# nimiq/snark-setup

Measured on NVIDIA B200. Metric: phase1 contribute+verify G1+G2 powers/sec at 2^22 (1/2/4/8 B200), bit-exact, higher is better.
Workload: dtype u32

## Files before the change

snark-setup_b200/csrc/fp.cuh:

```cuda
#pragma once
#include "ptx.cuh"

namespace ss {

template <class P>
struct Fp {
    static constexpr int N = P::N;
    using Params = P;
#ifndef SS_CALL_GROUP_OPS_LIMBS
#define SS_CALL_GROUP_OPS_LIMBS 12
#endif
    static constexpr bool CALL_GROUP_OPS = (N > SS_CALL_GROUP_OPS_LIMBS);
    uint32_t l[N];

    SS_HD static Fp zero() {
        Fp r;
#pragma unroll
        for (int i = 0; i < N; i++) r.l[i] = 0;
        return r;
    }
    SS_HD static Fp one() {
        Fp r;
#pragma unroll
        for (int i = 0; i < N; i++) r.l[i] = P::one(i);
        return r;
    }
    SS_HD bool is_zero() const {
        uint32_t t = 0;
#pragma unroll
        for (int i = 0; i < N; i++) t |= l[i];
        return t == 0;
    }
    SS_HD bool operator==(const Fp& o) const {
        uint32_t t = 0;
#pragma unroll
        for (int i = 0; i < N; i++) t |= l[i] ^ o.l[i];
        return t == 0;
    }
    SS_HD bool operator!=(const Fp& o) const { return !(*this == o); }
};

#if defined(__CUDACC__)
static __device__ __constant__ uint32_t kOpaqueOnes = 0xffffffffu;
#else
static const uint32_t kOpaqueOnes = 0xffffffffu;
#endif
SS_HD uint32_t opaque_neg(uint32_t x) { return (x ^ kOpaqueOnes) + 1u; }
#if defined(SS_NO_P0_TRICK)
#define SS_P0_TRICK false
#else
#define SS_P0_TRICK true
#endif

template <class P>
SS_HD void fp_final_sub(uint32_t* a) {
    constexpr int N = P::N;
    uint32_t t[N];
    t[0] = sub_cc(a[0], P::mod(0));
#pragma unroll
    for (int i = 1; i < N; i++) t[i] = subc_cc(a[i], P::mod(i));
    uint32_t borrow = subc(0, 0);
#pragma unroll
    for (int i = 0; i < N; i++) a[i] = borrow ? a[i] : t[i];
}

template <class P>
SS_HD Fp<P> fp_add(const Fp<P>& a, const Fp<P>& b) {
    constexpr int N = P::N;
    Fp<P> r;
    r.l[0] = add_cc(a.l[0], b.l[0]);
#pragma unroll
    for (int i = 1; i < N - 1; i++) r.l[i] = addc_cc(a.l[i], b.l[i]);
    r.l[N - 1] = addc(a.l[N - 1], b.l[N - 1]);
    fp_final_sub<P>(r.l);
    return r;
}

template <class P>
SS_HD Fp<P> fp_add_nr(const Fp<P>& a, const Fp<P>& b) {
    constexpr int N = P::N;
    Fp<P> r;
    r.l[0] = add_cc(a.l[0], b.l[0]);
#pragma unroll
    for (int i = 1; i < N - 1; i++) r.l[i] = addc_cc(a.l[i], b.l[i]);
    r.l[N - 1] = addc(a.l[N - 1], b.l[N - 1]);
    return r;
}

template <class P>
SS_HD Fp<P> fp_sub(const Fp<P>& a, const Fp<P>& b) {
    constexpr int N = P::N;
    Fp<P> r;
    r.l[0] = sub_cc(a.l[0], b.l[0]);
#pragma unroll
    for (int i = 1; i < N; i++) r.l[i] = subc_cc(a.l[i], b.l[i]);
    uint32_t borrow = subc(0, 0);
    r.l[0] = add_cc(r.l[0], P::mod(0) & borrow);
#pragma unroll
    for (int i = 1; i < N - 1; i++) r.l[i] = addc_cc(r.l[i], P::mod(i) & borrow);
    r.l[N - 1] = addc(r.l[N - 1], P::mod(N - 1) & borrow);
    return r;
}

template <class P>
SS_HD Fp<P> fp_neg(const Fp<P>& a) {
    constexpr int N = P::N;
    Fp<P> r;
    uint32_t nz = a.is_zero() ? 0u : 0xffffffffu;
    r.l[0] = sub_cc(P::mod(0), a.l[0]);
#pragma unroll
    for (int i = 1; i < N - 1; i++) r.l[i] = subc_cc(P::mod(i), a.l[i]);
    r.l[N - 1] = subc(P::mod(N - 1), a.l[N - 1]);
#pragma unroll
    for (int i = 0; i < N; i++) r.l[i] &= nz;
    return r;
}

template <class P>
SS_HD Fp<P> fp_dbl(const Fp<P>& a) {
    return fp_add(a, a);
}

template <class P>
SS_HD void mont_reduce_step(uint32_t* X, uint32_t* Y) {
    constexpr int N = P::N;
    constexpr bool P0_ONE = SS_P0_TRICK && (P::mod(0) == 1u);
    uint32_t m = P0_ONE ? opaque_neg(X[0]) : mul_lo(X[0], P::inv());
    Y[0] = mad_lo_cc(P::mod(1), m, Y[0]);
    Y[1] = madc_hi_cc(P::mod(1), m, Y[1]);
#pragma unroll
    for (int j = 2; j < N - 2; j += 2) {
        Y[j] = madc_lo_cc(P::mod(j + 1), m, Y[j]);
        Y[j + 1] = madc_hi_cc(P::mod(j + 1), m, Y[j + 1]);
    }
    Y[N - 2] = madc_lo_cc(P::mod(N - 1), m, Y[N - 2]);
    Y[N - 1] = madc_hi(P::mod(N - 1), m, Y[N - 1]);
    if (P0_ONE) {
        X[0] = add_cc(X[0], m);
        X[1] = addc_cc(X[1], 0);
    } else {
        X[0] = mad_lo_cc(P::mod(0), m, X[0]);
        X[1] = madc_hi_cc(P::mod(0), m, X[1]);
    }
#pragma unroll
    for (int j = 2; j < N; j += 2) {
        X[j] = madc_lo_cc(P::mod(j), m, X[j]);
        X[j + 1] = madc_hi_cc(P::mod(j), m, X[j + 1]);
    }
    Y[N - 1] = addc(Y[N - 1], 0);
}

template <class P>
SS_HD void mont_step(uint32_t* X , uint32_t* Y , const uint32_t* a, uint32_t bi) {
    constexpr int N = P::N;
    X[0] = add_cc(X[0], Y[1]);
#pragma unroll
    for (int j = 0; j < N - 2; j += 2) {
        Y[j] = madc_lo_cc(a[j + 1], bi, Y[j + 2]);
        Y[j + 1] = madc_hi_cc(a[j + 1], bi, Y[j + 3]);
    }
    Y[N - 2] = madc_lo_cc(a[N - 1], bi, 0);
    Y[N - 1] = madc_hi(a[N - 1], bi, 0);
    X[0] = mad_lo_cc(a[0], bi, X[0]);
    X[1] = madc_hi_cc(a[0], bi, X[1]);
#pragma unroll
    for (int j = 2; j < N; j += 2) {
        X[j] = madc_lo_cc(a[j], bi, X[j]);
        X[j + 1] = madc_hi_cc(a[j], bi, X[j + 1]);
    }
    Y[N - 1] = addc(Y[N - 1], 0);
    mont_reduce_step<P>(X, Y);
}

template <class P>
SS_HD Fp<P> fp_mul_inl(const Fp<P>& a, const Fp<P>& b) {
    constexpr int N = P::N;
    static_assert(N % 2 == 0, "even limb count");
    uint32_t X[N], Y[N];
#pragma unroll
    for (int j = 0; j < N; j += 2) {
        X[j] = mul_lo(a.l[j], b.l[0]);
        X[j + 1] = mul_hi(a.l[j], b.l[0]);
        Y[j] = mul_lo(a.l[j + 1], b.l[0]);
        Y[j + 1] = mul_hi(a.l[j + 1], b.l[0]);
    }
    mont_reduce_step<P>(X, Y);
#pragma unroll
    for (int i = 1; i < N; i += 2) {
        mont_step<P>(Y, X, a.l, b.l[i]);
        if (i + 1 < N) mont_step<P>(X, Y, a.l, b.l[i + 1]);
    }
    Fp<P> r;
    r.l[0] = add_cc(X[0], Y[1]);
#pragma unroll
    for (int j = 1; j < N - 1; j++) r.l[j] = addc_cc(X[j], Y[j + 1]);
    r.l[N - 1] = addc(X[N - 1], 0);
    fp_final_sub<P>(r.l);
    return r;
}

template <class P, int K>
SS_HD void fp_mul_xk_inl(const Fp<P> (&a)[K], const Fp<P> (&b)[K], Fp<P> (&r)[K]) {
    constexpr int N = P::N;
    static_assert(N % 2 == 0, "even limb count");
    uint32_t X[K][N], Y[K][N];
#pragma unroll
    for (int k = 0; k < K; k++) {
#pragma unroll
        for (int j = 0; j < N; j += 2) {
            X[k][j] = mul_lo(a[k].l[j], b[k].l[0]);
            X[k][j + 1] = mul_hi(a[k].l[j], b[k].l[0]);
            Y[k][j] = mul_lo(a[k].l[j + 1], b[k].l[0]);
            Y[k][j + 1] = mul_hi(a[k].l[j + 1], b[k].l[0]);
        }
    }
#pragma unroll
    for (int k = 0; k < K; k++) mont_reduce_step<P>(X[k], Y[k]);
#pragma unroll
    for (int i = 1; i < N; i += 2) {
#pragma unroll
        for (int k = 0; k < K; k++) mont_step<P>(Y[k], X[k], a[k].l, b[k].l[i]);
        if (i + 1 < N) {
#pragma unroll
            for (int k = 0; k < K; k++) mont_step<P>(X[k], Y[k], a[k].l, b[k].l[i + 1]);
        }
    }
#pragma unroll
    for (int k = 0; k < K; k++) {
        r[k].l[0] = add_cc(X[k][0], Y[k][1]);
#pragma unroll
        for (int j = 1; j < N - 1; j++) r[k].l[j] = addc_cc(X[k][j], Y[k][j + 1]);
        r[k].l[N - 1] = addc(X[k][N - 1], 0);
        fp_final_sub<P>(r[k].l);
    }
}

template <class P>
SS_HD void mont_row_acc(uint32_t* X, uint32_t* Y, const uint32_t* c, uint32_t di) {
    constexpr int N = P::N;
    Y[0] = mad_lo_cc(c[1], di, Y[0]);
    Y[1] = madc_hi_cc(c[1], di, Y[1]);
#pragma unroll
    for (int j = 2; j < N - 2; j += 2) {
        Y[j] = madc_lo_cc(c[j + 1], di, Y[j]);
        Y[j + 1] = madc_hi_cc(c[j + 1], di, Y[j + 1]);
    }
    Y[N - 2] = madc_lo_cc(c[N - 1], di, Y[N - 2]);
    Y[N - 1] = madc_hi(c[N - 1], di, Y[N - 1]);
    X[0] = mad_lo_cc(c[0], di, X[0]);
    X[1] = madc_hi_cc(c[0], di, X[1]);
#pragma unroll
    for (int j = 2; j < N; j += 2) {
        X[j] = madc_lo_cc(c[j], di, X[j]);
        X[j + 1] = madc_hi_cc(c[j], di, X[j + 1]);
    }
    Y[N - 1] = addc(Y[N - 1], 0);
}

template <class P>
SS_HD void mont_row_shift(uint32_t* X , uint32_t* Y , const uint32_t* a, uint32_t bi) {
    constexpr int N = P::N;
    X[0] = add_cc(X[0], Y[1]);
#pragma unroll
    for (int j = 0; j < N - 2; j += 2) {
        Y[j] = madc_lo_cc(a[j + 1], bi, Y[j + 2]);
        Y[j + 1] = madc_hi_cc(a[j + 1], bi, Y[j + 3]);
    }
    Y[N - 2] = madc_lo_cc(a[N - 1], bi, 0);
    Y[N - 1] = madc_hi(a[N - 1], bi, 0);
    X[0] = mad_lo_cc(a[0], bi, X[0]);
    X[1] = madc_hi_cc(a[0], bi, X[1]);
#pragma unroll
    for (int j = 2; j < N; j += 2) {
        X[j] = madc_lo_cc(a[j], bi, X[j]);
        X[j + 1] = madc_hi_cc(a[j], bi, X[j + 1]);
    }
    Y[N - 1] = addc(Y[N - 1], 0);
}

template <class P>
SS_HD Fp<P> fp_mul2_inl(const Fp<P>& a, const Fp<P>& b, const Fp<P>& c, const Fp<P>& d) {
    constexpr int N = P::N;
    uint32_t X[N], Y[N];
#pragma unroll
    for (int j = 0; j < N; j += 2) {
        X[j] = mul_lo(a.l[j], b.l[0]);
        X[j + 1] = mul_hi(a.l[j], b.l[0]);
        Y[j] = mul_lo(a.l[j + 1], b.l[0]);
        Y[j + 1] = mul_hi(a.l[j + 1], b.l[0]);
    }
    mont_row_acc<P>(X, Y, c.l, d.l[0]);
    mont_reduce_step<P>(X, Y);
#pragma unroll
    for (int i = 1; i < N; i += 2) {
        mont_row_shift<P>(Y, X, a.l, b.l[i]);
        mont_row_acc<P>(Y, X, c.l, d.l[i]);
        mont_reduce_step<P>(Y, X);
        if (i + 1 < N) {
            mont_row_shift<P>(X, Y, a.l, b.l[i + 1]);
            mont_row_acc<P>(X, Y, c.l, d.l[i + 1]);
            mont_reduce_step<P>(X, Y);
        }
    }
    Fp<P> r;
    r.l[0] = add_cc(X[0], Y[1]);
#pragma unroll
    for (int j = 1; j < N - 1; j++) r.l[j] = addc_cc(X[j], Y[j + 1]);
    r.l[N - 1] = addc(X[N - 1], 0);
    fp_final_sub<P>(r.l);
    return r;
}

#if defined(__CUDACC__)
template <class P>
__device__ __noinline__ Fp<P> fp_mul2_call(Fp<P> a, Fp<P> b, Fp<P> c, Fp<P> d) {
    return fp_mul2_inl(a, b, c, d);
}
#endif


template <class P>
SS_HD void mont_redc_shift_step(uint32_t* X , uint32_t* Y ) {
    constexpr int N = P::N;
    constexpr bool P0_ONE = SS_P0_TRICK && (P::mod(0) == 1u);
    uint32_t m = P0_ONE ? opaque_neg(X[0] + Y[1]) : mul_lo(X[0] + Y[1], P::inv());
    X[0] = add_cc(X[0], Y[1]);
#pragma unroll
    for (int j = 0; j < N - 2; j += 2) {
        Y[j] = madc_lo_cc(P::mod(j + 1), m, Y[j + 2]);
        Y[j + 1] = madc_hi_cc(P::mod(j + 1), m, Y[j + 3]);
    }
    Y[N - 2] = madc_lo_cc(P::mod(N - 1), m, 0);
    Y[N - 1] = madc_hi(P::mod(N - 1), m, 0);
    if (P0_ONE) {
        X[0] = add_cc(X[0], m);
        X[1] = addc_cc(X[1], 0);
    } else {
        X[0] = mad_lo_cc(P::mod(0), m, X[0]);
        X[1] = madc_hi_cc(P::mod(0), m, X[1]);
    }
#pragma unroll
    for (int j = 2; j < N; j += 2) {
        X[j] = madc_lo_cc(P::mod(j), m, X[j]);
        X[j + 1] = madc_hi_cc(P::mod(j), m, X[j + 1]);
    }
    Y[N - 1] = addc(Y[N - 1], 0);
}

template <class P>
SS_HD Fp<P> mont_redc_wide(uint32_t* E) {
    constexpr int N = P::N;
    uint32_t* X = E;
    uint32_t Y[N];
#pragma unroll
    for (int k = 0; k < N; k++) Y[k] = 0;
    mont_reduce_step<P>(X, Y);
#pragma unroll
    for (int i = 1; i < N; i += 2) {
        mont_redc_shift_step<P>(Y, X);
        if (i + 1 < N) mont_redc_shift_step<P>(X, Y);
    }
    Fp<P> r;
    r.l[0] = add_cc(X[0], Y[1]);
#pragma unroll
    for (int j = 1; j < N - 1; j++) r.l[j] = addc_cc(X[j], Y[j + 1]);
    r.l[N - 1] = addc(X[N - 1], 0);
    r.l[0] = add_cc(r.l[0], E[N]);
#pragma unroll
    for (int j = 1; j < N - 1; j++) r.l[j] = addc_cc(r.l[j], E[N + j]);
    r.l[N - 1] = addc(r.l[N - 1], E[2 * N - 1]);
    fp_final_sub<P>(r.l);
    return r;
}

#if defined(__CUDACC__)
template <class P>
__device__ __noinline__ Fp<P> fp_mul_call(Fp<P> a, Fp<P> b) {
    return fp_mul_inl(a, b);
}
#endif

#if defined(SS_COUNT_OPS) && !defined(__CUDACC__)
inline unsigned long long ss_op_count[3][32] = {};
#define SS_COUNT_OP(kind, n) (++ss_op_count[kind][n])
#else
#define SS_COUNT_OP(kind, n) ((void)0)
#endif

template <class P>
SS_HD Fp<P> fp_mul(const Fp<P>& a, const Fp<P>& b) {
#if defined(__CUDA_ARCH__) && !defined(SS_MUL_INLINE) && !defined(SS_MULONLY_INLINE)
    return fp_mul_call<P>(a, b);
#else
    SS_COUNT_OP(0, P::N);
    return fp_mul_inl(a, b);
#endif
}

template <class P>
SS_HD Fp<P> fp_mul2(const Fp<P>& a, const Fp<P>& b, const Fp<P>& c, const Fp<P>& d) {
#if defined(__CUDA_ARCH__) && !defined(SS_MUL_INLINE)
    return fp_mul2_call<P>(a, b, c, d);
#else
    SS_COUNT_OP(0, P::N);
    SS_COUNT_OP(2, P::N);
    return fp_mul2_inl(a, b, c, d);
#endif
}

template <class P>
SS_HD Fp<P> fp_sqr_inl(const Fp<P>& av) {
    constexpr int N = P::N;
    const uint32_t* a = av.l;
    uint32_t E[2 * N], O[2 * N];
#pragma unroll
    for (int k = 0; k < 2 * N; k++) E[k] = O[k] = 0;
#pragma unroll
    for (int i = 0; i < N - 1; i++) {
        {
            int last = -1;
#pragma unroll
            for (int j = i + 1; j < N; j += 2) {
                const int p = i + j;
                O[p - 1] = (j == i + 1) ? mad_lo_cc(a[i], a[j], O[p - 1]) : madc_lo_cc(a[i], a[j], O[p - 1]);
                O[p] = madc_hi_cc(a[i], a[j], O[p]);
                last = p;
            }
            if (last >= 0) O[last + 1] = addc(O[last + 1], 0);
        }
        {
            int last = -1;
#pragma unroll
            for (int j = i + 2; j < N; j += 2) {
                const int p = i + j;
                E[p] = (j == i + 2) ? mad_lo_cc(a[i], a[j], E[p]) : madc_lo_cc(a[i], a[j], E[p]);
                E[p + 1] = madc_hi_cc(a[i], a[j], E[p + 1]);
                last = p;
            }
            if (last >= 0) E[last + 2] = addc(E[last + 2], 0);
        }
    }
    E[1] = add_cc(E[1], O[0]);
#pragma unroll
    for (int k = 2; k < 2 * N - 1; k++) E[k] = addc_cc(E[k], O[k - 1]);
    E[2 * N - 1] = addc(E[2 * N - 1], O[2 * N - 2]);
    E[0] = add_cc(E[0], E[0]);
#pragma unroll
    for (int k = 1; k < 2 * N - 1; k++) E[k] = addc_cc(E[k], E[k]);
    E[2 * N - 1] = addc(E[2 * N - 1], E[2 * N - 1]);
    E[0] = mad_lo_cc(a[0], a[0], E[0]);
    E[1] = madc_hi_cc(a[0], a[0], E[1]);
#pragma unroll
    for (int i = 1; i < N - 1; i++) {
        E[2 * i] = madc_lo_cc(a[i], a[i], E[2 * i]);
        E[2 * i + 1] = madc_hi_cc(a[i], a[i], E[2 * i + 1]);
    }
    E[2 * N - 2] = madc_lo_cc(a[N - 1], a[N - 1], E[2 * N - 2]);
    E[2 * N - 1] = madc_hi(a[N - 1], a[N - 1], E[2 * N - 1]);
    return mont_redc_wide<P>(E);
}

#if defined(__CUDACC__)
template <class P>
__device__ __noinline__ Fp<P> fp_sqr_call(Fp<P> a) {
    return fp_sqr_inl(a);
}
#endif

template <class P>
SS_HD Fp<P> fp_sqr(const Fp<P>& a) {
#if defined(SS_NO_DEDICATED_SQR)
    return fp_mul(a, a);
#elif defined(__CUDA_ARCH__) && !defined(SS_MUL_INLINE) && !defined(SS_SQR_INLINE)
    return fp_sqr_call<P>(a);
#else
    SS_COUNT_OP(1, P::N);
    return fp_sqr_inl(a);
#endif
}

template <class P>
SS_HD Fp<P> fp_to_mont(const Fp<P>& a) {
    Fp<P> r2;
#pragma unroll
    for (int i = 0; i < P::N; i++) r2.l[i] = P::r2(i);
    return fp_mul(a, r2);
}

template <class P>
SS_HD Fp<P> fp_from_mont(const Fp<P>& a) {
    Fp<P> o = Fp<P>::zero();
    o.l[0] = 1;
    return fp_mul(a, o);
}

template <class P, class E, int W = 4>
SS_HD Fp<P> fp_pow(const Fp<P>& a, E exp_limb, int nlimbs) {
    constexpr int T = 1 << (W - 1);
    auto bit = [&](int i) -> uint32_t { return (exp_limb(i >> 5) >> (i & 31)) & 1u; };
    int i = 32 * nlimbs - 1;
    while (i >= 0 && !bit(i)) i--;
    if (i < 0) return Fp<P>::one();
    Fp<P> tab[T];
    tab[0] = a;
    {
        const Fp<P> a2 = fp_sqr(a);
#pragma unroll 1
        for (int k = 1; k < T; k++) tab[k] = fp_mul(tab[k - 1], a2);
    }
    Fp<P> r = a;
    bool started = false;
    while (i >= 0) {
        if (!bit(i)) {
            r = fp_sqr(r);
            i--;
            continue;
        }
        int j = i - W + 1;
        if (j < 0) j = 0;
        while (!bit(j)) j++;
        uint32_t v = 0;
        for (int k = i; k >= j; k--) v = (v << 1) | bit(k);
        if (started) {
#pragma unroll 1
            for (int k = 0; k < i - j + 1; k++) r = fp_sqr(r);
            r = fp_mul(r, tab[v >> 1]);
        } else {
            r = tab[v >> 1];
            started = true;
        }
        i = j - 1;
    }
    return r;
}

template <int W, class P, class E>
SS_HD Fp<P> fp_pow_win(const Fp<P>& a, E exp_limb, int nlimbs) {
    return fp_pow<P, E, W>(a, exp_limb, nlimbs);
}

template <class P>
SS_HD Fp<P> fp_inv(const Fp<P>& a) {
    return fp_pow<P>(a, [](int i) { return P::pm2(i); }, P::N);
}

template <int N>
SS_HD bool raw_gt(const uint32_t* a, const uint32_t* b) {
    uint32_t t = sub_cc(b[0], a[0]);
#pragma unroll
    for (int i = 1; i < N; i++) t = subc_cc(b[i], a[i]);
    (void)t;
    return subc(0, 0) != 0;
}

template <class P>
SS_HD bool raw_ge_mod(const uint32_t* a) {
    uint32_t t = sub_cc(a[0], P::mod(0));
#pragma unroll
    for (int i = 1; i < P::N; i++) t = subc_cc(a[i], P::mod(i));
    (void)t;
    return subc(0, 0) == 0;
}

template <class P>
SS_HD bool fp_sqrt(const Fp<P>& a, Fp<P>& out) {
    if (a.is_zero()) {
        out = a;
        return true;
    }
    if (P::P3MOD4) {
        Fp<P> r = fp_pow<P>(a, [](int i) { return P::pp1q(i); }, P::N);
        out = r;
        return fp_sqr(r) == a;
    } else {
        Fp<P> w = fp_pow<P>(a, [](int i) { return P::tm1h(i); }, P::N);
        Fp<P> x = fp_mul(a, w);
        Fp<P> b = fp_mul(x, w);
        Fp<P> z;
#pragma unroll
        for (int i = 0; i < P::N; i++) z.l[i] = P::root_of_unity(i);
        const Fp<P> one = Fp<P>::one();
        int v = P::TWO_ADICITY;
        while (!(b == one)) {
            int k = 0;
            Fp<P> b2k = b;
            while (!(b2k == one)) {
                b2k = fp_sqr(b2k);
                k++;
                if (k == v) return false;
            }
            Fp<P> wj = z;
            for (int j = 0; j < v - k - 1; j++) wj = fp_sqr(wj);
            z = fp_sqr(wj);
            b = fp_mul(b, z);
            x = fp_mul(x, wj);
            v = k;
        }
        out = x;
        return true;
    }
}

}
```

snark-setup_b200/csrc/fp2.cuh:

```cuda
#pragma once
#include "constants_gen.cuh"
#include "fp.cuh"

namespace ss {

template <class P>
struct Fp2Config {
    static constexpr int NR = -5;
};
template <>
struct Fp2Config<Mnt753Q> {
    static constexpr int NR = 13;
};

template <class P>
SS_HD Fp<P> fp_mul_small(const Fp<P>& x, unsigned k) {
    Fp<P> r = Fp<P>::zero();
    bool started = false;
    for (int b = 31; b >= 0; b--) {
        if (started) r = fp_dbl(r);
        if ((k >> b) & 1u) {
            r = started ? fp_add(r, x) : x;
            started = true;
        }
    }
    return r;
}
template <class P>
SS_HD Fp<P> fp_mul_nr(const Fp<P>& x) {
    constexpr int NR = Fp2Config<P>::NR;
    Fp<P> m = fp_mul_small(x, (unsigned)(NR < 0 ? -NR : NR));
    return NR < 0 ? fp_neg(m) : m;
}

template <class P>
struct Fp2 {
    using Base = Fp<P>;
    using Params = P;
    static constexpr bool CALL_GROUP_OPS = true;
    Base c0, c1;

    SS_HD static Fp2 zero() { return Fp2{Base::zero(), Base::zero()}; }
    SS_HD static Fp2 one() { return Fp2{Base::one(), Base::zero()}; }
    SS_HD bool is_zero() const { return c0.is_zero() && c1.is_zero(); }
    SS_HD bool operator==(const Fp2& o) const { return c0 == o.c0 && c1 == o.c1; }
    SS_HD bool operator!=(const Fp2& o) const { return !(*this == o); }
};

template <class P>
SS_HD Fp<P> fp_mul5(const Fp<P>& x) {
    Fp<P> t = fp_dbl(fp_dbl(x));
    return fp_add(t, x);
}

template <class P>
SS_HD Fp2<P> fp_add(const Fp2<P>& a, const Fp2<P>& b) {
    return Fp2<P>{fp_add(a.c0, b.c0), fp_add(a.c1, b.c1)};
}
template <class P>
SS_HD Fp2<P> fp_sub(const Fp2<P>& a, const Fp2<P>& b) {
    return Fp2<P>{fp_sub(a.c0, b.c0), fp_sub(a.c1, b.c1)};
}
template <class P>
SS_HD Fp2<P> fp_neg(const Fp2<P>& a) {
    return Fp2<P>{fp_neg(a.c0), fp_neg(a.c1)};
}
template <class P>
SS_HD Fp2<P> fp_dbl(const Fp2<P>& a) {
    return Fp2<P>{fp_dbl(a.c0), fp_dbl(a.c1)};
}

#ifndef SS_FP2_UNITS
#define SS_FP2_UNITS 0
#endif
template <class P>
SS_HD Fp2<P> fp2_mul_body(const Fp2<P>& a, const Fp2<P>& b) {
    const Fp<P> x[3] = {a.c0, a.c1, fp_add_nr(a.c0, a.c1)};
    const Fp<P> y[3] = {b.c0, b.c1, fp_add_nr(b.c0, b.c1)};
    Fp<P> v[3];
    fp_mul_xk_inl<P, 3>(x, y, v);
    Fp2<P> r;
    r.c1 = fp_sub(fp_sub(v[2], v[0]), v[1]);
    r.c0 = fp_sub(v[0], fp_mul5(v[1]));
    return r;
}
template <class P>
SS_HD Fp2<P> fp2_sqr_body(const Fp2<P>& a) {
    const Fp<P> x[2] = {a.c0, fp_add_nr(a.c0, a.c1)};
    const Fp<P> y[2] = {a.c1, fp_sub(a.c0, fp_mul5(a.c1))};
    Fp<P> v[2];
    fp_mul_xk_inl<P, 2>(x, y, v);
    const Fp<P> v2 = fp_dbl(v[0]);
    Fp2<P> r;
    r.c0 = fp_add(v[1], fp_dbl(v2));
    r.c1 = v2;
    return r;
}
#if defined(__CUDACC__)
template <class P>
__device__ __noinline__ Fp2<P> fp2_mul_call(Fp2<P> a, Fp2<P> b) {
    return fp2_mul_body(a, b);
}
template <class P>
__device__ __noinline__ Fp2<P> fp2_sqr_call(Fp2<P> a) {
    return fp2_sqr_body(a);
}
#endif
template <class P>
constexpr bool kFp2Units = SS_FP2_UNITS && Fp2Config<P>::NR == -5 && P::N <= 12;

template <class P>
SS_HD Fp2<P> fp_mul(const Fp2<P>& a, const Fp2<P>& b) {
#if defined(__CUDA_ARCH__) && !defined(SS_MUL_INLINE)
    if constexpr (kFp2Units<P>) return fp2_mul_call<P>(a, b);
#endif
    Fp<P> v0 = fp_mul(a.c0, b.c0);
    Fp<P> v1 = fp_mul(a.c1, b.c1);
#if defined(SS_FP2_REDUCED_SUMS)
    Fp<P> s = fp_mul(fp_add(a.c0, a.c1), fp_add(b.c0, b.c1));
#else
    Fp<P> s = fp_mul(fp_add_nr(a.c0, a.c1), fp_add_nr(b.c0, b.c1));
#endif
    Fp2<P> r;
    r.c1 = fp_sub(fp_sub(s, v0), v1);
    if constexpr (Fp2Config<P>::NR == -5) r.c0 = fp_sub(v0, fp_mul5(v1));
    else r.c0 = fp_add(v0, fp_mul_nr(v1));
    return r;
}

template <class P>
SS_HD Fp2<P> fp_sqr(const Fp2<P>& a) {
#if defined(__CUDA_ARCH__) && !defined(SS_MUL_INLINE)
    if constexpr (kFp2Units<P>) return fp2_sqr_call<P>(a);
#endif
    if constexpr (Fp2Config<P>::NR != -5) {
        Fp<P> v = fp_mul(a.c0, a.c1);
        Fp<P> t = fp_mul(fp_add(a.c0, a.c1), fp_add(a.c0, fp_mul_nr(a.c1)));
        constexpr int K = Fp2Config<P>::NR + 1;
        Fp<P> kv = fp_mul_small(v, (unsigned)(K < 0 ? -K : K));
        return Fp2<P>{K < 0 ? fp_add(t, kv) : fp_sub(t, kv), fp_dbl(v)};
    }
    Fp<P> v = fp_mul(a.c0, a.c1);
#if defined(SS_FP2_REDUCED_SUMS)
    Fp<P> t = fp_mul(fp_add(a.c0, a.c1), fp_sub(a.c0, fp_mul5(a.c1)));
#else
    Fp<P> t = fp_mul(fp_add_nr(a.c0, a.c1), fp_sub(a.c0, fp_mul5(a.c1)));
#endif
    Fp<P> v2 = fp_dbl(v);
    Fp2<P> r;
    r.c0 = fp_add(t, fp_dbl(v2));
    r.c1 = v2;
    return r;
}

template <class P>
SS_HD Fp2<P> fp_mul_base(const Fp2<P>& a, const Fp<P>& k) {
    return Fp2<P>{fp_mul(a.c0, k), fp_mul(a.c1, k)};
}

template <class P>
SS_HD Fp2<P> fp_inv(const Fp2<P>& a) {
    Fp<P> n = fp_sub(fp_sqr(a.c0), fp_mul_nr(fp_sqr(a.c1)));
    Fp<P> ni = fp_inv(n);
    return Fp2<P>{fp_mul(a.c0, ni), fp_neg(fp_mul(a.c1, ni))};
}

template <class P>
SS_HD bool fp_sqrt(const Fp2<P>& a, Fp2<P>& out) {
    if (a.c1.is_zero()) {
        Fp<P> r;
        if (fp_sqrt(a.c0, r)) {
            out = Fp2<P>{r, Fp<P>::zero()};
            return true;
        }
        Fp<P> q = fp_mul(a.c0, fp_inv(fp_mul_nr(Fp<P>::one())));
        if (!fp_sqrt(q, r)) return false;
        out = Fp2<P>{Fp<P>::zero(), r};
        return true;
    }
    Fp<P> norm = fp_sub(fp_sqr(a.c0), fp_mul_nr(fp_sqr(a.c1)));
    Fp<P> alpha;
    if (!fp_sqrt(norm, alpha)) return false;
    Fp<P> half;
#pragma unroll
    for (int i = 0; i < P::N; i++) half.l[i] = P::half(i);
    Fp<P> delta = fp_mul(fp_add(a.c0, alpha), half);
    Fp<P> c0;
    if (!fp_sqrt(delta, c0)) {
        delta = fp_mul(fp_sub(a.c0, alpha), half);
        if (!fp_sqrt(delta, c0)) return false;
    }
    Fp<P> c1 = fp_mul(a.c1, fp_inv(fp_dbl(c0)));
    out = Fp2<P>{c0, c1};
    return true;
}


template <class P>
struct Fp3 {
    using Base = Fp<P>;
    using Params = P;
    static constexpr bool CALL_GROUP_OPS = true;
    static constexpr unsigned NR = 11;
    Base c0, c1, c2;

    SS_HD static Fp3 zero() { return Fp3{Base::zero(), Base::zero(), Base::zero()}; }
    SS_HD static Fp3 one() { return Fp3{Base::one(), Base::zero(), Base::zero()}; }
    SS_HD bool is_zero() const { return c0.is_zero() && c1.is_zero() && c2.is_zero(); }
    SS_HD bool operator==(const Fp3& o) const { return c0 == o.c0 && c1 == o.c1 && c2 == o.c2; }
    SS_HD bool operator!=(const Fp3& o) const { return !(*this == o); }
};
template <class P>
SS_HD Fp3<P> fp_add(const Fp3<P>& a, const Fp3<P>& b) { return Fp3<P>{fp_add(a.c0, b.c0), fp_add(a.c1, b.c1), fp_add(a.c2, b.c2)}; }
template <class P>
SS_HD Fp3<P> fp_sub(const Fp3<P>& a, const Fp3<P>& b) { return Fp3<P>{fp_sub(a.c0, b.c0), fp_sub(a.c1, b.c1), fp_sub(a.c2, b.c2)}; }
template <class P>
SS_HD Fp3<P> fp_neg(const Fp3<P>& a) { return Fp3<P>{fp_neg(a.c0), fp_neg(a.c1), fp_neg(a.c2)}; }
template <class P>
SS_HD Fp3<P> fp_dbl(const Fp3<P>& a) { return Fp3<P>{fp_dbl(a.c0), fp_dbl(a.c1), fp_dbl(a.c2)}; }
#if defined(__CUDACC__)
template <class P>
__device__ __host__ __noinline__
#else
template <class P>
inline
#endif
Fp3<P> fp3_mul_impl(const Fp3<P>& a, const Fp3<P>& b) {
    constexpr unsigned NR = Fp3<P>::NR;
    Fp3<P> r;
    r.c0 = fp_add(fp_mul(a.c0, b.c0), fp_mul_small(fp_add(fp_mul(a.c1, b.c2), fp_mul(a.c2, b.c1)), NR));
    r.c1 = fp_add(fp_add(fp_mul(a.c0, b.c1), fp_mul(a.c1, b.c0)), fp_mul_small(fp_mul(a.c2, b.c2), NR));
    r.c2 = fp_add(fp_add(fp_mul(a.c0, b.c2), fp_mul(a.c1, b.c1)), fp_mul(a.c2, b.c0));
    return r;
}
template <class P>
SS_HD Fp3<P> fp_mul(const Fp3<P>& a, const Fp3<P>& b) { return fp3_mul_impl(a, b); }
template <class P>
SS_HD Fp3<P> fp_sqr(const Fp3<P>& a) { return fp3_mul_impl(a, a); }
template <class P>
SS_HD Fp3<P> fp_inv(const Fp3<P>& a) {
    constexpr unsigned NR = Fp3<P>::NR;
    Fp<P> t0 = fp_sub(fp_sqr(a.c0), fp_mul_small(fp_mul(a.c1, a.c2), NR));
    Fp<P> t1 = fp_sub(fp_mul_small(fp_sqr(a.c2), NR), fp_mul(a.c0, a.c1));
    Fp<P> t2 = fp_sub(fp_sqr(a.c1), fp_mul(a.c0, a.c2));
    Fp<P> d = fp_add(fp_mul(a.c0, t0), fp_mul_small(fp_add(fp_mul(a.c2, t1), fp_mul(a.c1, t2)), NR));
    Fp<P> di = fp_inv(d);
    return Fp3<P>{fp_mul(t0, di), fp_mul(t1, di), fp_mul(t2, di)};
}
template <class P, class SQ>
SS_HD bool fp3_sqrt(const Fp3<P>& a, Fp3<P>& out) {
    if (a.is_zero()) {
        out = a;
        return true;
    }
    Fp3<P> w = Fp3<P>::one();
    bool started = false;
    for (int i = SQ::TM1H_LIMBS - 1; i >= 0; i--) {
        const uint32_t e = SQ::tm1h(i);
        for (int b = 31; b >= 0; b--) {
            if (started) w = fp_sqr(w);
            if ((e >> b) & 1u) {
                w = started ? fp_mul(w, a) : a;
                started = true;
            }
        }
    }
    if (!started) w = Fp3<P>::one();
    Fp3<P> x = fp_mul(a, w);
    Fp3<P> b = fp_mul(x, w);
    Fp3<P> z;
#pragma unroll
    for (int i = 0; i < P::N; i++) {
        z.c0.l[i] = SQ::z_c0(i);
        z.c1.l[i] = SQ::z_c1(i);
        z.c2.l[i] = SQ::z_c2(i);
    }
    const Fp3<P> one = Fp3<P>::one();
    int v = SQ::TWO_ADICITY;
    while (!(b == one)) {
        int k = 0;
        Fp3<P> b2k = b;
        while (!(b2k == one)) {
            b2k = fp_sqr(b2k);
            k++;
            if (k == v) return false;
        }
        Fp3<P> wj = z;
        for (int j = 0; j < v - k - 1; j++) wj = fp_sqr(wj);
        z = fp_sqr(wj);
        b = fp_mul(b, z);
        x = fp_mul(x, wj);
        v = k;
    }
    out = x;
    return true;
}

}
```

Before: 1.376 million.

## Use lazy Montgomery reduction for Fp2 multiplication with nonresidue -5

Adds an Fp2 multiply that computes the three Karatsuba products as unreduced double-width values. It combines them in wide form, adding 20·p² to keep c0 = T0 − 5·T1 non-negative, and runs only two Montgomery reductions instead of three. This is meant to remove one reduction and several modular add/sub corrections per Fp2 mul, at the cost of more register pressure from wide temporaries. It is enabled by default when the existing Fp2 unit path is not taken and the field has enough headroom bits.

```diff
diff --git a/snark-setup_b200/csrc/fp.cuh b/snark-setup_b200/csrc/fp.cuh
--- a/snark-setup_b200/csrc/fp.cuh
+++ b/snark-setup_b200/csrc/fp.cuh
@@ -373,6 +373,95 @@
     return r;
 }
 
+template <class P>
+SS_HD void fp_mul_wide_inl(const Fp<P>& av, const Fp<P>& bv, uint32_t* T ) {
+    constexpr int N = P::N;
+    const uint32_t* a = av.l;
+    const uint32_t* b = bv.l;
+    uint32_t* E = T;
+    uint32_t O[2 * N - 1];
+#pragma unroll
+    for (int k = 0; k < 2 * N; k++) E[k] = 0;
+#pragma unroll
+    for (int k = 0; k < 2 * N - 1; k++) O[k] = 0;
+#pragma unroll
+    for (int i = 0; i < N; i++) {
+        {
+            int last = -1;
+#pragma unroll
+            for (int j = i & 1; j < N; j += 2) {
+                const int p = i + j;
+                E[p] = (j == (i & 1)) ? mad_lo_cc(a[i], b[j], E[p]) : madc_lo_cc(a[i], b[j], E[p]);
+                if (p + 2 < 2 * N) E[p + 1] = madc_hi_cc(a[i], b[j], E[p + 1]);
+                else E[p + 1] = madc_hi(a[i], b[j], E[p + 1]);
+                last = p;
+            }
+            if (last + 2 < 2 * N) E[last + 2] = addc(E[last + 2], 0);
+        }
+        {
+            int last = -1;
+#pragma unroll
+            for (int j = 1 - (i & 1); j < N; j += 2) {
+                const int p = i + j;
+                O[p - 1] = (j == 1 - (i & 1)) ? mad_lo_cc(a[i], b[j], O[p - 1]) : madc_lo_cc(a[i], b[j], O[p - 1]);
+                O[p] = madc_hi_cc(a[i], b[j], O[p]);
+                last = p;
+            }
+            O[last + 1] = addc(O[last + 1], 0);
+        }
+    }
+    E[1] = add_cc(E[1], O[0]);
+#pragma unroll
+    for (int k = 2; k < 2 * N - 1; k++) E[k] = addc_cc(E[k], O[k - 1]);
+    E[2 * N - 1] = addc(E[2 * N - 1], O[2 * N - 2]);
+}
+
+template <int M>
+SS_HD void wide_add(uint32_t* x, const uint32_t* y) {
+    x[0] = add_cc(x[0], y[0]);
+#pragma unroll
+    for (int k = 1; k < M - 1; k++) x[k] = addc_cc(x[k], y[k]);
+    x[M - 1] = addc(x[M - 1], y[M - 1]);
+}
+template <int M>
+SS_HD void wide_sub(uint32_t* x, const uint32_t* y) {
+    x[0] = sub_cc(x[0], y[0]);
+#pragma unroll
+    for (int k = 1; k < M - 1; k++) x[k] = subc_cc(x[k], y[k]);
+    x[M - 1] = subc(x[M - 1], y[M - 1]);
+}
+template <int M, int S>
+SS_HD void wide_sub_shl(uint32_t* x, const uint32_t* y) {
+    static_assert(S > 0 && S < 32, "shift");
+    x[0] = sub_cc(x[0], y[0] << S);
+#pragma unroll
+    for (int k = 1; k < M - 1; k++) x[k] = subc_cc(x[k], (y[k] << S) | (y[k - 1] >> (32 - S)));
+    x[M - 1] = subc(x[M - 1], (y[M - 1] << S) | (y[M - 2] >> (32 - S)));
+}
+
+template <class P, unsigned K>
+struct WideMultipleP2 {
+    uint32_t v[2 * P::N];
+    constexpr WideMultipleP2() : v() {
+        constexpr int N = P::N;
+        for (int i = 0; i < N; i++) {
+            uint64_t c = 0;
+            for (int j = 0; j < N; j++) {
+                const uint64_t t = (uint64_t)P::mod(i) * P::mod(j) + v[i + j] + c;
+                v[i + j] = (uint32_t)t;
+                c = t >> 32;
+            }
+            v[i + N] = (uint32_t)c;
+        }
+        uint64_t c = 0;
+        for (int k = 0; k < 2 * N; k++) {
+            const uint64_t t = (uint64_t)v[k] * K + c;
+            v[k] = (uint32_t)t;
+            c = t >> 32;
+        }
+    }
+};
+
 #if defined(__CUDACC__)
 template <class P>
 __device__ __noinline__ Fp<P> fp_mul_call(Fp<P> a, Fp<P> b) {
@@ -381,7 +470,7 @@
 #endif
 
 #if defined(SS_COUNT_OPS) && !defined(__CUDACC__)
-inline unsigned long long ss_op_count[3][32] = {};
+inline unsigned long long ss_op_count[4][32] = {};
 #define SS_COUNT_OP(kind, n) (++ss_op_count[kind][n])
 #else
 #define SS_COUNT_OP(kind, n) ((void)0)
diff --git a/snark-setup_b200/csrc/fp2.cuh b/snark-setup_b200/csrc/fp2.cuh
--- a/snark-setup_b200/csrc/fp2.cuh
+++ b/snark-setup_b200/csrc/fp2.cuh
@@ -109,11 +109,52 @@
 template <class P>
 constexpr bool kFp2Units = SS_FP2_UNITS && Fp2Config<P>::NR == -5 && P::N <= 12;
 
+#ifndef SS_FP2_LAZY
+#define SS_FP2_LAZY 1
+#endif
+template <class P>
+constexpr bool kFp2Lazy = SS_FP2_LAZY && Fp2Config<P>::NR == -5 && P::BITS + 5 <= 32 * P::N;
+template <class P>
+SS_HD Fp2<P> fp2_mul_lazy_body(const Fp2<P>& a, const Fp2<P>& b) {
+    constexpr int M = 2 * P::N;
+    constexpr WideMultipleP2<P, 20> K20{};
+    const Fp<P> sa = fp_add_nr(a.c0, a.c1), sb = fp_add_nr(b.c0, b.c1);
+    uint32_t T0[M], T1[M], D[M];
+    fp_mul_wide_inl<P>(a.c0, b.c0, T0);
+    fp_mul_wide_inl<P>(a.c1, b.c1, T1);
+#pragma unroll
+    for (int k = 0; k < M; k++) D[k] = T0[k];
+    wide_add<M>(D, T1);
+    wide_add<M>(T0, K20.v);
+    wide_sub_shl<M, 2>(T0, T1);
+    wide_sub<M>(T0, T1);
+    Fp2<P> r;
+    r.c0 = mont_redc_wide<P>(T0);
+    fp_mul_wide_inl<P>(sa, sb, T0);
+    wide_sub<M>(T0, D);
+    r.c1 = mont_redc_wide<P>(T0);
+    return r;
+}
+#if defined(__CUDACC__)
+template <class P>
+__device__ __noinline__ Fp2<P> fp2_mul_lazy_call(Fp2<P> a, Fp2<P> b) {
+    return fp2_mul_lazy_body(a, b);
+}
+#endif
+
 template <class P>
 SS_HD Fp2<P> fp_mul(const Fp2<P>& a, const Fp2<P>& b) {
 #if defined(__CUDA_ARCH__) && !defined(SS_MUL_INLINE)
     if constexpr (kFp2Units<P>) return fp2_mul_call<P>(a, b);
-#endif
+    if constexpr (kFp2Lazy<P>) return fp2_mul_lazy_call<P>(a, b);
+#endif
+    if constexpr (kFp2Lazy<P>) {
+        SS_COUNT_OP(0, P::N);
+        SS_COUNT_OP(0, P::N);
+        SS_COUNT_OP(0, P::N);
+        SS_COUNT_OP(3, P::N);
+        return fp2_mul_lazy_body(a, b);
+    }
     Fp<P> v0 = fp_mul(a.c0, b.c0);
     Fp<P> v1 = fp_mul(a.c1, b.c1);
 #if defined(SS_FP2_REDUCED_SUMS)
```

After: 1.400 million (median of 6 runs). 1.8% higher.
